# rawahars/CS744-Distributed-Data-Parallel

Hardware: AMD Instinct MI355X
Metric: images/sec (whole node) VGG-11 CIFAR-shaped at 1/2/4/8 MI355X; scaling eff (higher is better)
Workload: dtype fp32; 1 GPU; model=VGG-11, global_batch=256, local_batch=256, parallelism=dp1, comm=none, backend=native, device=mi355x, hipgraph=True, optimizer=SGD(lr=0.1, momentum=0.9, wd=1e-4), optimizer_overlap=False, early_buffer_broadcast=False, conv_gemm=f16x2

## Files before the change

### csrc/kernels/bwd_pair.h

```cpp
#pragma once
#include "conv_x3_body.h"
#include "wgrad_x3_body.h"

namespace cdp {
namespace pair_detail {

using namespace x3conv;
using namespace x3wgrad;

template <int DBM, int DBN, int WBM, int WBN>
struct PairCfg {
  static constexpr int kThreads = waves_m<DBM>() * 128;
  static_assert(kThreads == wg_threads<WBM>(), "both bodies must run the same workgroup size");
  static constexpr int kSmem = conv_x3_smem_elems<DBM, DBN, 2>() > wgrad_x3_smem_elems<WBM, WBN, 2, true>()
                                   ? conv_x3_smem_elems<DBM, DBN, 2>()
                                   : wgrad_x3_smem_elems<WBM, WBN, 2, true>();
};

template <int DBM, int DBN, int WBM, int WBN>
__global__ __launch_bounds__(waves_m<DBM>() * 128, DBM >= 256 ? 1 : 2) void bwd_pair_kernel(
    ConvGemmParams pd, WgradParams pw, int nd, int nw) {
  __shared__ __attribute__((aligned(16))) __bf16 smem[PairCfg<DBM, DBN, WBM, WBN>::kSmem];
  const int b = blockIdx.x;
  if (b < nd) conv_x3_body<DBM, DBN, 0, true, 2>(pd, smem, b, nd);
  else wgrad_x3_body<WBM, WBN, true, 2, true>(pw, smem, b - nd, nw);
}

template <int DBM, int DBN, int WBM, int WBN>
void launch_pair(const ConvGemmParams& pd, const WgradParams& pw, hipStream_t st) {
  const int nd = ((pd.M + DBM - 1) / DBM) * ((pd.Nout + DBN - 1) / DBN) * pd.splits;
  const int nw = ((pw.Cout + WBM - 1) / WBM) * ((pw.Kdim + WBN - 1) / WBN) * pw.splits;
  hipLaunchKernelGGL((bwd_pair_kernel<DBM, DBN, WBM, WBN>), dim3(nd + nw), dim3(PairCfg<DBM, DBN, WBM, WBN>::kThreads),
                     0, st, pd, pw, nd, nw);
}

template <int DBM, int DBN>
bool launch_pair_d(int wbm, int wbn, const ConvGemmParams& pd, const WgradParams& pw, hipStream_t st);
template <>
bool launch_pair_d<128, 128>(int, int, const ConvGemmParams&, const WgradParams&, hipStream_t);
template <>
bool launch_pair_d<128, 64>(int, int, const ConvGemmParams&, const WgradParams&, hipStream_t);
template <>
bool launch_pair_d<64, 128>(int, int, const ConvGemmParams&, const WgradParams&, hipStream_t);
template <>
bool launch_pair_d<64, 64>(int, int, const ConvGemmParams&, const WgradParams&, hipStream_t);

}
}

#define CDP_PAIR_TU(DBM, DBN)                                                                              \
  namespace cdp {                                                                                          \
  namespace pair_detail {                                                                                  \
  template <>                                                                                              \
  bool launch_pair_d<DBM, DBN>(int wbm, int wbn, const ConvGemmParams& pd, const WgradParams& pw,          \
                               hipStream_t st) {                                                           \
    if (wbm == 128 && wbn == 128) launch_pair<DBM, DBN, 128, 128>(pd, pw, st);                             \
    else if (wbm == 128 && wbn == 64) launch_pair<DBM, DBN, 128, 64>(pd, pw, st);                          \
    else if (wbm == 64 && wbn == 128) launch_pair<DBM, DBN, 64, 128>(pd, pw, st);                          \
    else if (wbm == 64 && wbn == 64) launch_pair<DBM, DBN, 64, 64>(pd, pw, st);                            \
    else return false;                                                                                     \
    return true;                                                                                           \
  }                                                                                                        \
  }                                                                                                        \
  }
```

### csrc/kernels/bwd_pair.hip

```cpp
#include "bwd_pair.h"

namespace cdp {

bool bwd_pair_ok(const ConvGemmParams& pd, int bm, int bn, const WgradParams& pw, int wbm, int wbn, int np) {
  if (np != 2 || (pd.C % 32) != 0 || (pd.Kdim % 32) != 0 || (pw.C % 4) != 0 || (pw.Cout % 4) != 0) return false;
  if (bm == 256) return bn == 128 && wbm == 256 && wbn == 128;
  return (bm == 64 || bm == 128) && (bn == 64 || bn == 128) && (wbm == 64 || wbm == 128) && (wbn == 64 || wbn == 128);
}

void bwd_pair_launch(const ConvGemmParams& pd, int bm, int bn, const WgradParams& pw, int wbm, int wbn,
                     hipStream_t st) {
  using namespace pair_detail;
  bool ok = false;
  if (bm == 256) {
    launch_pair<256, 128, 256, 128>(pd, pw, st);
    ok = true;
  } else if (bm == 128 && bn == 128) ok = launch_pair_d<128, 128>(wbm, wbn, pd, pw, st);
  else if (bm == 128 && bn == 64) ok = launch_pair_d<128, 64>(wbm, wbn, pd, pw, st);
  else if (bm == 64 && bn == 128) ok = launch_pair_d<64, 128>(wbm, wbn, pd, pw, st);
  else if (bm == 64 && bn == 64) ok = launch_pair_d<64, 64>(wbm, wbn, pd, pw, st);
  (void)ok;
}

}
```

### csrc/kernels/conv_x3.hip

```cpp
#include "conv_x3_body.h"

namespace cdp {

namespace {

using namespace x3conv;

template <int BM, int BN, int MODE, bool DGRAD, int NP = 3>
__global__ __launch_bounds__(waves_m<BM>() * 128, (NP == 2 && BM + BN <= 256) ? 2 : (BM + BN >= 256) ? 1 : 2) void
conv_x3_kernel(ConvGemmParams p) {
  __shared__ __attribute__((aligned(16))) __bf16 smem[conv_x3_smem_elems<BM, BN, NP>()];
  conv_x3_body<BM, BN, MODE, DGRAD, NP>(p, smem, blockIdx.x, gridDim.x);
}

template <int BM, int BN, int MODE, bool DGRAD>
void launch_x3(const ConvGemmParams& p, int ntiles, int np, hipStream_t st) {
  const dim3 blk(waves_m<BM>() * 128), grd(ntiles * p.splits);
  if (np == 1) hipLaunchKernelGGL((conv_x3_kernel<BM, BN, MODE, DGRAD, 1>), grd, blk, 0, st, p);
  else if (np == 2) hipLaunchKernelGGL((conv_x3_kernel<BM, BN, MODE, DGRAD, 2>), grd, blk, 0, st, p);
  else hipLaunchKernelGGL((conv_x3_kernel<BM, BN, MODE, DGRAD, 3>), grd, blk, 0, st, p);
}

template <int MODE, bool DGRAD>
void dispatch_x3(const ConvGemmParams& p, int bm, int bn, int np, hipStream_t st) {
  const int ntm = (p.M + bm - 1) / bm, ntn = (p.Nout + bn - 1) / bn;
  const int nt = ntm * ntn;
  if (bm == 256) launch_x3<256, 128, MODE, DGRAD>(p, nt, np, st);
  else if (bm == 128 && bn == 128) launch_x3<128, 128, MODE, DGRAD>(p, nt, np, st);
  else if (bm == 128 && bn == 64) launch_x3<128, 64, MODE, DGRAD>(p, nt, np, st);
  else if (bm == 64 && bn == 128) launch_x3<64, 128, MODE, DGRAD>(p, nt, np, st);
  else launch_x3<64, 64, MODE, DGRAD>(p, nt, np, st);
}

}

void conv_x3_launch(const ConvGemmParams& p, int bm, int bn, bool dgrad, hipStream_t st, int np) {
  if ((p.C % BK) == 0 && (p.Kdim % BK) == 0) {
    if (dgrad) dispatch_x3<0, true>(p, bm, bn, np, st);
    else dispatch_x3<0, false>(p, bm, bn, np, st);
  } else if ((p.C % 4) == 0 && (p.Kdim % 4) == 0) {
    if (dgrad) dispatch_x3<1, true>(p, bm, bn, np, st);
    else dispatch_x3<1, false>(p, bm, bn, np, st);
  } else {
    if (dgrad) dispatch_x3<2, true>(p, bm, bn, np, st);
    else dispatch_x3<2, false>(p, bm, bn, np, st);
  }
}

}
```

### csrc/kernels/conv_x3_body.h

```cpp
#pragma once
#include <type_traits>

#include "common.h"
#include "conv_epilogue.h"
#include "kernels.h"
#include "x3_common.h"

namespace cdp {
namespace x3conv {

constexpr int BK = 32;
constexpr int LDH = BK;

__device__ __forceinline__ int chunk_pos(int r, int c) { return c ^ ((-(r >> 2)) & 3); }

__device__ __forceinline__ void split8(const float (&v)[8], u32x4& s0, u32x4& s1, u32x4& s2) {
#pragma unroll
  for (int j = 0; j < 4; ++j) {
    unsigned a, b, c;
    split_pair(v[2 * j], v[2 * j + 1], a, b, c);
    s0[j] = a;
    s1[j] = b;
    s2[j] = c;
  }
// ... 1 lines not shown

__device__ __forceinline__ void split8h(const float (&v)[8], float s, u32x4& s0, u32x4& s1) {
#pragma unroll
  for (int j = 0; j < 4; ++j) {
    unsigned a, b;
    split_pair_h(v[2 * j], v[2 * j + 1], s, a, b);
    s0[j] = a;
    s1[j] = b;
  }
}

__device__ __forceinline__ u32x4 pack8(const float (&v)[8]) {
  u32x4 r;
#pragma unroll
  for (int j = 0; j < 4; ++j) r[j] = pack_bf16x2(f32x2{v[2 * j], v[2 * j + 1]});
  return r;
}

template <int BM, int BN, int NP>
constexpr int conv_x3_scales_at() {
  return 2 * NP * (BM + BN) * LDH > 2 * epi_lds_floats<BM, BN>() ? 2 * NP * (BM + BN) * LDH
                                                                  : 2 * epi_lds_floats<BM, BN>();
}
template <int BM, int BN, int NP>
constexpr int conv_x3_smem_elems() {
  return conv_x3_scales_at<BM, BN, NP>() + (NP == 2 ? 2 * (BM + BN) : 0);
}

template <int BM, int BN, int MODE, bool DGRAD, int NP = 3>
__device__ __forceinline__ void conv_x3_body(const ConvGemmParams& p, __bf16* __restrict__ smem, int vbid, int nvb) {
  static_assert(NP >= 1 && NP <= 3, "planes");
  constexpr unsigned ES = 2u;
  constexpr int WM = waves_m<BM>();
  constexpr int NT = WM * 128;
  constexpr int RS = NT / 4;
  constexpr int TM = BM / WM / 32;
  constexpr int TN = BN / 64;
  constexpr int A_LD = BM / RS;
  constexpr int B_LD = BN / RS;
  static_assert(A_LD >= 1 && B_LD >= 1, "tile too narrow for the loader");
  constexpr int PA = BM * LDH, PB = BN * LDH;
  constexpr int STAGE = NP * (PA + PB);

  const int tid = threadIdx.x;
  const int lane = tid & 63;
  const int wid = tid >> 6;
  const int wm = wid >> 1, wn = wid & 1;

  const int ntn = (p.Nout + BN - 1) / BN;
  const int bid = xcd_remap(vbid, nvb);
  const int tn_idx = bid % ntn;
  const int rest = bid / ntn;
  const int split = rest % p.splits;
  const int tm_idx = rest / p.splits;
// ... 321 lines not shown
      __syncthreads();
    }
    if (kt < kt_end) compute(smem);
  } else {
    finish_scales();
    publish_scales();
    __syncthreads();
  }

  if constexpr (NP == 2) {
#pragma unroll
    for (int b = 0; b < TN; ++b) {
      const float ib = s_ib[wn * (BN / 2) + b * 32 + l32];
#pragma unroll
      for (int a = 0; a < TM; ++a)
#pragma unroll
        for (int r = 0; r < 16; ++r)
          acc[a][b][r] = acc[a][b][r] * s_ia[wm * (BM / WM) + a * 32 + (r & 3) + 8 * (r >> 2) + 4 * hh] * ib;
    }
  }
  conv_epilogue<BM, BN>(p, acc, reinterpret_cast<float*>(smem), m0, n0, tm_idx, split);
}

}
}
```

### csrc/kernels/kernels.h

```cpp
#pragma once
#include <hip/hip_runtime.h>

#include "erase.h"
#include "lars.h"
#include "lr_sched.h"
#include "mix.h"
#include "rrc.h"

namespace cdp {

struct FastDiv {
  unsigned d, mul, shift;
};

inline FastDiv make_fastdiv(int d) {
  FastDiv f{(unsigned)d, 0u, 0u};
  if (d <= 1) return f;
  unsigned l = 0;
  while ((1ull << l) < (unsigned long long)d) ++l;
  const unsigned long long p = 31ull + l;
  f.mul = (unsigned)(((1ull << p) + (unsigned long long)d - 1ull) / (unsigned long long)d);
  f.shift = (unsigned)(p - 32ull);
  return f;
}
// ... 42 lines not shown

struct WgradParams {
  const float* dy;
  const float* x;
  float* out;
  int N, H, W, C, P, Q, KH, KW, stride, pad;
  int Cout, Kdim, M, splits;
  FastDiv fd_PQ, fd_Q, fd_C, fd_KW;
  const unsigned* dy_ch;
  const unsigned* x_ch;
};

constexpr int kActCopies = 8;
struct ActMaxOut {
  unsigned* img;
  unsigned* ch;
};
inline long long act_max_elems(long long N, long long C) { return N + kActCopies * C; }
inline long long weight_max_elems(long long Co, long long Ci) {
  return ((Ci + 31) / 32) * Co + ((Co + 31) / 32) * Ci;
}

void conv_igemm_launch(const ConvGemmParams& p, int bm, int bn, bool dgrad, hipStream_t st);
void conv_x3_launch(const ConvGemmParams& p, int bm, int bn, bool dgrad, hipStream_t st, int np = 3);
void splitk_reduce_launch(const float* slab, int S, int M, int Nout, const float* bias, float* y, float* part,
                          hipStream_t st, const RowRemap* rr = nullptr, const float* addend = nullptr);
int splitk_rows_per_part();

void wgrad_launch(const WgradParams& p, int bm, int bn, bool x3, hipStream_t st, int np = 3);
void act_max_launch(const float* x, int N, long long HW, int C, ActMaxOut o, hipStream_t st);
constexpr int kMaxAmaxSegs = 64;
struct WeightPrepArgs {
  const float* w[kMaxAmaxSegs];
  float* wt[kMaxAmaxSegs];
  int co[kMaxAmaxSegs], t[kMaxAmaxSegs], ci[kMaxAmaxSegs];
  int blk0[kMaxAmaxSegs + 1];
  long long pofs[kMaxAmaxSegs];
  int nseg;
};
void weight_prep_launch(const WeightPrepArgs& a, float* part, hipStream_t st);
struct SgdPrepSeg {
  long long off;
  float* wt;
  int co, t, ci, blk0;
  long long pofs;
};
struct SgdPrepChunk {
// ... 16 lines not shown
  long long* state = nullptr;
  const LrSchedCfg* cfg = nullptr;
  float* last_lr = nullptr;
  int advance = 0;
};
void sgd_prep_launch(float* p, const float* g, float* buf, const SgdPrepSeg* segs, int nseg, int nblk_w,
                     const SgdPrepChunk* chunks, int nchunk, float* wmax, const float* lr_ptr, float lr,
                     float momentum, float dampening, float wd, float grad_scale, bool nesterov, bool first,
                     bool maximize, hipStream_t st, long long* counter = nullptr, const ClipArgs& clip = ClipArgs{},
                     const LarsArgs& lars = LarsArgs{}, const EmaArgs& ema = EmaArgs{},
                     const SchedArgs& sched = SchedArgs{});
void slab_sum_launch(const float* slab, int S, long long n, float* dst, bool accumulate, hipStream_t st);
void slab_sum_strided_launch(const float* slab, int S, long long n_src, int src_cols, int dst_cols, float* dst,
                             bool accumulate, hipStream_t st);

bool stem_ok(int Cin, int KH, int KW, int stride, int pad, int Co);
void stem_fwd_launch(const float* x, const float* w, const float* bias, float* y, float* part, int N, int H, int W,
                     int Cin, int Co, hipStream_t st);
int stem_wgrad_blocks(int N, int H, int W);
void stem_wgrad_launch(const float* y, const float* gout, const float* stats, const float* sums, const float* x,
                       float* slab, int nblk, int N, int H, int W, int Cin, hipStream_t st);

bool bwd_pair_ok(const ConvGemmParams& pd, int bm, int bn, const WgradParams& pw, int wbm, int wbn, int np);
void bwd_pair_launch(const ConvGemmParams& pd, int bm, int bn, const WgradParams& pw, int wbm, int wbn,
                     hipStream_t st);

struct BwdReduceArgs {
  const float* d_slab;
  float* d_y;
  const float* d_addend;
  int d_S, d_M, d_Nout;
  const float* bn_y;
  const float* bn_stats;
  float* bn_part;
  int bn_H, bn_W, bn_pool, bn_relu, bn_ps;
  FastDiv bn_fd_wo, bn_fd_ho;
  const float4* w_slab;
  float4* w_dst;
  int w_S;
  long long w_n4;
  int nbd, d_nbx, w_cb;
};
void bwd_reduce_launch(BwdReduceArgs a, hipStream_t st);
int bwd_reduce_rows_per_part();

int bn_bwd_grid(int N, int H, int W, int C, bool pool);
void bn_finalize_launch(const float* part, int nparts, int rpp, int M, int C, const float* gamma, const float* beta,
                        float* running_mean, float* running_var, long long* nbt, float momentum, float eps,
// ... 119 lines not shown
```

### csrc/runtime/bindings.cpp

```cpp
#include <torch/csrc/utils/pybind.h>
#include <torch/extension.h>

#include <execinfo.h>
#include <signal.h>
#include <unistd.h>

#include "ops.h"
#include "rccl_comm.h"
#include "reducer.h"

namespace py = pybind11;
using namespace cdp;

namespace {
void segv_backtrace(int sig) {
  void* frames[64];
  const int n = backtrace(frames, 64);
  const char msg[] = "[cdp] native backtrace:\n";
  (void)!write(2, msg, sizeof(msg) - 1);
  backtrace_symbols_fd(frames, n, 2);
  signal(sig, SIG_DFL);
  raise(sig);
}
}

PYBIND11_MODULE(_C, m) {
  if (const char* bt = std::getenv("CDP_SEGV_BT"); bt && bt[0] == '1') signal(SIGSEGV, segv_backtrace);
  m.doc() = "cs744_distributed_data_parallel_amd native runtime (gfx950 kernels, RCCL comm, reducer)";
  m.attr("ARCH") = "gfx950";

  m.def("set_conv_gemm", &set_conv_gemm, py::arg("mode"),
        "select the conv GEMM engine: x3 (3-term bf16 split), f16x2 (scaled 2-term fp16 split), f32 (exact fp32 "
        "MFMA) or bf16 (bf16 operands, non-parity)");
  m.def("get_conv_gemm", &get_conv_gemm);
  m.def("set_gemm_override", &set_gemm_override, py::arg("kind"), py::arg("bm") = 0, py::arg("bn") = 0,
        py::arg("splits") = 0, "force the tile / split-K plan of later GEMMs (tuning sweeps; zeros restore the planner)");
  m.def("pair_launches", &pair_launches, "paired data/weight-gradient launches issued so far");
  m.def("plan_info", &plan_info, py::arg("kind"), py::arg("M"), py::arg("N"), py::arg("K"));
  m.def("clear_hip_error", [] { return std::string(hipGetErrorName(hipGetLastError())); },
        "reset the thread's last HIP error (e.g. after an invalidated stream capture) and return its name");
  m.def("conv2d_fwd", &conv2d_fwd, py::arg("x"), py::arg("w"), py::arg("bias"), py::arg("stride"), py::arg("pad"),
        py::arg("want_stats") = false, py::arg("x_amax") = py::none(), py::arg("w_amax") = py::none());
  m.def("conv2d_dgrad", &conv2d_dgrad, py::arg("dy"), py::arg("w"), py::arg("in_shape"), py::arg("stride"),
        py::arg("pad"), py::arg("addend") = py::none(), py::arg("dy_amax") = py::none(), py::arg("w_amax") = py::none(),
        py::arg("w_t") = py::none());
  m.def("conv2d_wgrad", &conv2d_wgrad, py::arg("dy"), py::arg("x"), py::arg("w_shape"), py::arg("stride"),
        py::arg("pad"), py::arg("out") = py::none(), py::arg("accumulate") = false, py::arg("dy_amax") = py::none(),
        py::arg("x_amax") = py::none());
  m.def("conv_bn_act_fwd", &conv_bn_act_fwd, py::arg("x"), py::arg("w"), py::arg("b"), py::arg("gamma"),
        py::arg("beta"), py::arg("running_mean"), py::arg("running_var"), py::arg("num_batches_tracked"),
        py::arg("momentum"), py::arg("eps"), py::arg("training"), py::arg("stride"), py::arg("pad"), py::arg("pool"),
        py::arg("relu"), py::arg("residual"), py::arg("x_amax") = py::none(), py::arg("w_amax") = py::none(),
        py::arg("res_y") = py::none(), py::arg("res_stats") = py::none(), py::arg("defer_apply") = false,
        "fused conv + BN [+ residual] [+ ReLU] [+ 2x2 max-pool] forward; returns (out, y, stats, x_saved, out_amax, "
        "x_amax, w_amax, relu_mask). defer_apply: statistics only, out a shape-only placeholder; res_y / res_stats: "
        "the residual as such a deferred branch's raw output and stats, normalized inside this block's apply pass");
  m.def("act_max", &act_max_of, py::arg("t"),
        "f16x2 engine: an activation's per-image / per-channel |max| slots by the standalone pass (int32 [N + "
        "copies * C], float bits; undefined tensor for other engines)");
  m.def("act_max_memsets", &act_max_memsets, "slot-chunk memsets issued so far (tests)");
// ... 266 lines not shown
```

### csrc/runtime/ops.cpp

```cpp
#include "ops.h"

#include <c10/hip/HIPCachingAllocator.h>
#include <c10/hip/HIPFunctions.h>
#include <c10/hip/HIPGuard.h>
#include <c10/hip/HIPStream.h>
#include <torch/extension.h>

#include <algorithm>
#include <array>
#include <atomic>
#include <cstdlib>
#include <cstring>
#include <functional>
#include <mutex>
#include <tuple>
#include <string>
#include <unordered_map>

#include "../kernels/adam.h"
#include "../kernels/kernels.h"

namespace cdp {

namespace {
// ... 352 lines not shown
  std::lock_guard<std::mutex> g(gemm_log_mu());
  gemm_log_vec().push_back({kind, M, N, K, bm, bn, splits});
}
std::vector<std::tuple<std::string, int64_t, int64_t, int64_t, int64_t, int64_t, int64_t>> gemm_log_snapshot(bool clear) {
  std::lock_guard<std::mutex> g(gemm_log_mu());
  std::vector<std::tuple<std::string, int64_t, int64_t, int64_t, int64_t, int64_t, int64_t>> out;
  for (const auto& r : gemm_log_vec()) out.emplace_back(r.kind, r.M, r.N, r.K, r.bm, r.bn, r.splits);
  if (clear) gemm_log_vec().clear();
  return out;
}
static void wgrad_launch_logged(const WgradParams& p, int bm, int bn, bool x3, hipStream_t st, int np) {
  gemm_log_add("wgrad", p.Cout, p.Kdim, (long long)p.M, bm, bn, p.splits);
  wgrad_launch(p, bm, bn, x3, st, np);
}

static bool narrow_stores() {
  static const bool on = [] {
    const char* e = std::getenv("CDP_WIDE_STORES");
    return e && e[0] == '0';
  }();
  return on;
}

void conv_launch(const ConvGemmParams& p0, int bm, int bn, bool dgrad, hipStream_t st) {
  gemm_log_add(dgrad ? "dgrad" : "fwd", p0.M, p0.Nout, p0.Kdim, bm, bn, p0.splits);
  ConvGemmParams p = p0;
  p.narrow = narrow_stores();
  if (x3_family() && x3_ok(p, dgrad)) {
    TORCH_CHECK(!f16x2_mode() || (p.a_img && p.b_row), "f16x2 conv GEMM launched without operand maxima");
    conv_x3_launch(p, bm, bn, dgrad, st, split_planes());
  }
  else conv_igemm_launch(p, bm, bn, dgrad, st);
}

struct DeferredReduce {
  at::Tensor w_slab;
  float* w_dst = nullptr;
  int w_S = 0;
  long long w_n = 0;
  at::Tensor d_slab;
  const float* d_src = nullptr;
  float* d_y = nullptr;
  const float* d_addend = nullptr;
  int d_S = 0, d_M = 0, d_Nout = 0;
  bool d_on = false;
};

struct PendingWgrad {
  bool set = false;
  WgradParams p{};
  int bm = 0, bn = 0;
  std::function<void()> after;
  std::vector<at::Tensor> keep;
// ... 17 lines not shown

bool bwd_fuse_enabled() {
  static const bool on = [] {
    const char* e = std::getenv("CDP_BWD_FUSE");
    return !(e && e[0] == '0');
  }();
  return on;
}

std::atomic<long long>& pair_counter() {
  static std::atomic<long long> n{0};
  return n;
}

void conv_launch_or_pair(const ConvGemmParams& p, const GemmPlan& g, bool dgrad, hipStream_t st,
                         PendingWgrad* pending) {
  if (pending && pending->set && dgrad && f16x2_mode() && x3_ok(p, true) && p.a_img && p.b_row &&
      bwd_pair_ok(p, g.bm, g.bn, pending->p, pending->bm, pending->bn, split_planes())) {
    gemm_log_add("pair_dgrad", p.M, p.Nout, p.Kdim, g.bm, g.bn, p.splits);
    gemm_log_add("pair_wgrad", pending->p.Cout, pending->p.Kdim, (long long)pending->p.M, pending->bm, pending->bn,
                 pending->p.splits);
    ConvGemmParams q = p;
    q.narrow = narrow_stores();
    bwd_pair_launch(q, g.bm, g.bn, pending->p, pending->bm, pending->bn, st);
    pair_counter().fetch_add(1, std::memory_order_relaxed);
    pending->run_after();
    return;
  }
  conv_launch(p, g.bm, g.bn, dgrad, st);
}

int conv_gemm_splitk(ConvGemmParams p, const GemmPlan& g, bool dgrad, hipStream_t st, at::TensorOptions opts,
                     std::vector<at::Tensor>& keep, const std::function<float*(int)>& alloc_part = nullptr,
                     DeferredReduce* defer = nullptr, PendingWgrad* pending = nullptr) {
  p.splits = g.splits;
  if (g.splits == 1) {
    if (alloc_part) p.part = alloc_part(g.bm);
    conv_launch_or_pair(p, g, dgrad, st, pending);
    if (defer && !alloc_part && !p.part && !p.bias && !p.rr.on && !p.addend && (p.Nout % 4) == 0) {
      defer->d_on = true;
      defer->d_src = p.y;
      defer->d_y = p.y;
      defer->d_addend = nullptr;
      defer->d_S = 1;
      defer->d_M = p.M;
      defer->d_Nout = p.Nout;
    }
    return g.bm;
// ... 309 lines not shown
}

at::Tensor pad_channels4(const at::Tensor& t, at::Tensor* amax = nullptr) {
  const int64_t C = t.size(1), C4 = (C + 3) / 4 * 4;
  at::Tensor o = at::empty({t.size(0), C4, t.size(2), t.size(3)}, t.options().memory_format(at::MemoryFormat::ChannelsLast));
  if (C < 4 && t.is_contiguous(at::MemoryFormat::ChannelsLast)) {
    hipStream_t st = cur_stream();
    ActMaxOut am{nullptr, nullptr};
    if (amax) {
      *amax = new_act_max(t.size(0), 4, t, st);
      am = act_out(*amax, t.size(0));
    }
    pad_c4_launch(t.data_ptr<float>(), (int)t.size(0), t.size(2) * t.size(3), (int)C, o.data_ptr<float>(), am, st);
    return o;
  }
  o.zero_();
  o.narrow(1, 0, C).copy_(t);
  return o;
}

}

int64_t pair_launches() { return pair_counter().load(std::memory_order_relaxed); }

void set_gemm_override(const std::string& kind, int64_t bm, int64_t bn, int64_t splits) {
  TORCH_CHECK(kind == "conv" || kind == "wgrad", "set_gemm_override: kind must be 'conv' or 'wgrad'");
  TORCH_CHECK(bm == 0 || bm == 64 || bm == 128 || bm == 256, "bm must be 0, 64, 128 or 256");
  TORCH_CHECK(bn == 0 || bn == 64 || bn == 128, "bn must be 0, 64 or 128");
  TORCH_CHECK(bm != 256 || bn == 128, "256-row tiles are 256x128");
  PlanOverride& o = kind == "conv" ? conv_override() : wgrad_override();
  o.bm = (int)bm;
  o.bn = (int)bn;
  o.splits = (int)splits;
}

std::vector<int64_t> plan_info(const std::string& kind, int64_t M, int64_t N, int64_t K) {
  if (kind == "conv" || kind == "dgrad") {
    const GemmPlan g = plan_gemm(M, (int)N, (int)K, kind == "dgrad" ? 1 : 0);
    return {g.bm, g.bn, g.splits};
  }
  TORCH_CHECK(kind == "wgrad", "plan_info: kind must be 'conv', 'dgrad' or 'wgrad'");
  const WgradPlan w = plan_wgrad((int)N, (int)K, M);
  return {w.bm, w.bn, w.splits};
}

void set_conv_gemm(const std::string& mode) {
// ... 1651 lines not shown
```

### csrc/runtime/ops.h

```cpp
#pragma once
#include <ATen/ATen.h>
#include <c10/util/Optional.h>

#include <string>
#include <tuple>
#include <vector>

namespace cdp {

void set_conv_gemm(const std::string& mode);
int64_t pair_launches();
void set_gemm_override(const std::string& kind, int64_t bm, int64_t bn, int64_t splits);
std::vector<int64_t> plan_info(const std::string& kind, int64_t M, int64_t N, int64_t K);
std::string get_conv_gemm();
std::vector<at::Tensor> conv2d_fwd(const at::Tensor& x, const at::Tensor& w, const c10::optional<at::Tensor>& bias,
                                   int64_t stride, int64_t pad, bool want_stats,
                                   const c10::optional<at::Tensor>& x_amax = c10::nullopt,
                                   const c10::optional<at::Tensor>& w_amax = c10::nullopt);
at::Tensor conv2d_dgrad(const at::Tensor& dy, const at::Tensor& w, std::vector<int64_t> in_shape, int64_t stride,
                        int64_t pad, const c10::optional<at::Tensor>& addend,
                        const c10::optional<at::Tensor>& dy_amax = c10::nullopt,
                        const c10::optional<at::Tensor>& w_amax = c10::nullopt,
                        const c10::optional<at::Tensor>& w_t = c10::nullopt);
at::Tensor conv2d_wgrad(const at::Tensor& dy, const at::Tensor& x, std::vector<int64_t> w_shape, int64_t stride,
                        int64_t pad, const c10::optional<at::Tensor>& out, bool accumulate,
                        const c10::optional<at::Tensor>& dy_amax = c10::nullopt,
                        const c10::optional<at::Tensor>& x_amax = c10::nullopt);
at::Tensor conv2d_wgrad_keep(const at::Tensor& dy, const at::Tensor& x, std::vector<int64_t> w_shape, int64_t stride,
                             int64_t pad, const c10::optional<at::Tensor>& out, bool accumulate, int64_t keep_c,
                             const c10::optional<at::Tensor>& dy_amax = c10::nullopt,
                             const c10::optional<at::Tensor>& x_amax = c10::nullopt);
std::vector<at::Tensor> conv_bn_act_fwd(const at::Tensor& x, const at::Tensor& w, const c10::optional<at::Tensor>& b,
                                        const c10::optional<at::Tensor>& gamma, const c10::optional<at::Tensor>& beta,
                                        const c10::optional<at::Tensor>& running_mean,
// ... 167 lines not shown
```

Baseline: 199,100 images/sec.

## Add tap-reuse main loop for 3x3 conv GEMMs on small feature maps

Adds a specialized conv main loop for 3x3 stride-1 pad-1 convolutions whose whole output image fits in an M tile. It loads each activation channel chunk into LDS once and reuses it across all nine filter taps by shifting rows, instead of re-gathering the im2col tile for every tap. The loop is wired into the plain conv launch and the paired dgrad/wgrad kernel, and is on by default where a heuristic says it pays. The cost is extra LDS for a zero row, a more complex tap/row indexing path, and added template instantiations.

Result: no change. 200,600 images/sec (median of 6 runs) (+0.8%).

```diff
diff --git a/csrc/kernels/bwd_pair.h b/csrc/kernels/bwd_pair.h
--- a/csrc/kernels/bwd_pair.h
+++ b/csrc/kernels/bwd_pair.h
@@ -8,42 +8,56 @@
 using namespace x3conv;
 using namespace x3wgrad;
 
-template <int DBM, int DBN, int WBM, int WBN>
+template <int DBM, int DBN, int WBM, int WBN, bool TR = false>
 struct PairCfg {
   static constexpr int kThreads = waves_m<DBM>() * 128;
   static_assert(kThreads == wg_threads<WBM>(), "both bodies must run the same workgroup size");
-  static constexpr int kSmem = conv_x3_smem_elems<DBM, DBN, 2>() > wgrad_x3_smem_elems<WBM, WBN, 2, true>()
-                                   ? conv_x3_smem_elems<DBM, DBN, 2>()
+  static constexpr int kSmem = conv_x3_smem_elems<DBM, DBN, 2, TR>() > wgrad_x3_smem_elems<WBM, WBN, 2, true>()
+                                   ? conv_x3_smem_elems<DBM, DBN, 2, TR>()
                                    : wgrad_x3_smem_elems<WBM, WBN, 2, true>();
 };
 
-template <int DBM, int DBN, int WBM, int WBN>
+template <int DBM, int DBN, int WBM, int WBN, bool TR = false>
 __global__ __launch_bounds__(waves_m<DBM>() * 128, DBM >= 256 ? 1 : 2) void bwd_pair_kernel(
     ConvGemmParams pd, WgradParams pw, int nd, int nw) {
-  __shared__ __attribute__((aligned(16))) __bf16 smem[PairCfg<DBM, DBN, WBM, WBN>::kSmem];
+  __shared__ __attribute__((aligned(16))) __bf16 smem[PairCfg<DBM, DBN, WBM, WBN, TR>::kSmem];
   const int b = blockIdx.x;
-  if (b < nd) conv_x3_body<DBM, DBN, 0, true, 2>(pd, smem, b, nd);
+  if (b < nd) conv_x3_body<DBM, DBN, 0, true, 2, TR>(pd, smem, b, nd);
   else wgrad_x3_body<WBM, WBN, true, 2, true>(pw, smem, b - nd, nw);
 }
 
-template <int DBM, int DBN, int WBM, int WBN>
+template <int DBM, int DBN, int WBM, int WBN, bool TR = false>
 void launch_pair(const ConvGemmParams& pd, const WgradParams& pw, hipStream_t st) {
   const int nd = ((pd.M + DBM - 1) / DBM) * ((pd.Nout + DBN - 1) / DBN) * pd.splits;
   const int nw = ((pw.Cout + WBM - 1) / WBM) * ((pw.Kdim + WBN - 1) / WBN) * pw.splits;
-  hipLaunchKernelGGL((bwd_pair_kernel<DBM, DBN, WBM, WBN>), dim3(nd + nw), dim3(PairCfg<DBM, DBN, WBM, WBN>::kThreads),
-                     0, st, pd, pw, nd, nw);
+  hipLaunchKernelGGL((bwd_pair_kernel<DBM, DBN, WBM, WBN, TR>), dim3(nd + nw),
+                     dim3(PairCfg<DBM, DBN, WBM, WBN, TR>::kThreads), 0, st, pd, pw, nd, nw);
 }
 
 template <int DBM, int DBN>
-bool launch_pair_d(int wbm, int wbn, const ConvGemmParams& pd, const WgradParams& pw, hipStream_t st);
+constexpr bool pair_tr_built() { return !(DBM == 128 && DBN == 64); }
+
+template <int DBM, int DBN, int WBM, int WBN>
+void launch_pair_tr(bool tr, const ConvGemmParams& pd, const WgradParams& pw, hipStream_t st) {
+  if constexpr (pair_tr_built<DBM, DBN>()) {
+    if (tr) {
+      launch_pair<DBM, DBN, WBM, WBN, true>(pd, pw, st);
+      return;
+    }
+  }
+  launch_pair<DBM, DBN, WBM, WBN>(pd, pw, st);
+}
+
+template <int DBM, int DBN>
+bool launch_pair_d(int wbm, int wbn, bool tr, const ConvGemmParams& pd, const WgradParams& pw, hipStream_t st);
 template <>
-bool launch_pair_d<128, 128>(int, int, const ConvGemmParams&, const WgradParams&, hipStream_t);
+bool launch_pair_d<128, 128>(int, int, bool, const ConvGemmParams&, const WgradParams&, hipStream_t);
 template <>
-bool launch_pair_d<128, 64>(int, int, const ConvGemmParams&, const WgradParams&, hipStream_t);
+bool launch_pair_d<128, 64>(int, int, bool, const ConvGemmParams&, const WgradParams&, hipStream_t);
 template <>
-bool launch_pair_d<64, 128>(int, int, const ConvGemmParams&, const WgradParams&, hipStream_t);
+bool launch_pair_d<64, 128>(int, int, bool, const ConvGemmParams&, const WgradParams&, hipStream_t);
 template <>
-bool launch_pair_d<64, 64>(int, int, const ConvGemmParams&, const WgradParams&, hipStream_t);
+bool launch_pair_d<64, 64>(int, int, bool, const ConvGemmParams&, const WgradParams&, hipStream_t);
 
 }
 }
@@ -52,12 +66,12 @@
   namespace cdp {                                                                                          \
   namespace pair_detail {                                                                                  \
   template <>                                                                                              \
-  bool launch_pair_d<DBM, DBN>(int wbm, int wbn, const ConvGemmParams& pd, const WgradParams& pw,          \
+  bool launch_pair_d<DBM, DBN>(int wbm, int wbn, bool tr, const ConvGemmParams& pd, const WgradParams& pw, \
                                hipStream_t st) {                                                           \
-    if (wbm == 128 && wbn == 128) launch_pair<DBM, DBN, 128, 128>(pd, pw, st);                             \
-    else if (wbm == 128 && wbn == 64) launch_pair<DBM, DBN, 128, 64>(pd, pw, st);                          \
-    else if (wbm == 64 && wbn == 128) launch_pair<DBM, DBN, 64, 128>(pd, pw, st);                          \
-    else if (wbm == 64 && wbn == 64) launch_pair<DBM, DBN, 64, 64>(pd, pw, st);                            \
+    if (wbm == 128 && wbn == 128) launch_pair_tr<DBM, DBN, 128, 128>(tr, pd, pw, st);                      \
+    else if (wbm == 128 && wbn == 64) launch_pair_tr<DBM, DBN, 128, 64>(tr, pd, pw, st);                   \
+    else if (wbm == 64 && wbn == 128) launch_pair_tr<DBM, DBN, 64, 128>(tr, pd, pw, st);                   \
+    else if (wbm == 64 && wbn == 64) launch_pair_tr<DBM, DBN, 64, 64>(tr, pd, pw, st);                     \
     else return false;                                                                                     \
     return true;                                                                                           \
   }                                                                                                        \
diff --git a/csrc/kernels/bwd_pair.hip b/csrc/kernels/bwd_pair.hip
--- a/csrc/kernels/bwd_pair.hip
+++ b/csrc/kernels/bwd_pair.hip
@@ -8,17 +8,20 @@
   return (bm == 64 || bm == 128) && (bn == 64 || bn == 128) && (wbm == 64 || wbm == 128) && (wbn == 64 || wbn == 128);
 }
 
+bool bwd_pair_has_tap_reuse(int bm, int bn) { return !(bm == 128 && bn == 64); }
+
 void bwd_pair_launch(const ConvGemmParams& pd, int bm, int bn, const WgradParams& pw, int wbm, int wbn,
-                     hipStream_t st) {
+                     hipStream_t st, bool tap_reuse) {
   using namespace pair_detail;
+  const bool tr = tap_reuse && bwd_pair_has_tap_reuse(bm, bn) && conv_tap_reuse_ok(pd, bm, true, 2);
   bool ok = false;
   if (bm == 256) {
-    launch_pair<256, 128, 256, 128>(pd, pw, st);
+    launch_pair_tr<256, 128, 256, 128>(tr, pd, pw, st);
     ok = true;
-  } else if (bm == 128 && bn == 128) ok = launch_pair_d<128, 128>(wbm, wbn, pd, pw, st);
-  else if (bm == 128 && bn == 64) ok = launch_pair_d<128, 64>(wbm, wbn, pd, pw, st);
-  else if (bm == 64 && bn == 128) ok = launch_pair_d<64, 128>(wbm, wbn, pd, pw, st);
-  else if (bm == 64 && bn == 64) ok = launch_pair_d<64, 64>(wbm, wbn, pd, pw, st);
+  } else if (bm == 128 && bn == 128) ok = launch_pair_d<128, 128>(wbm, wbn, tr, pd, pw, st);
+  else if (bm == 128 && bn == 64) ok = launch_pair_d<128, 64>(wbm, wbn, tr, pd, pw, st);
+  else if (bm == 64 && bn == 128) ok = launch_pair_d<64, 128>(wbm, wbn, tr, pd, pw, st);
+  else if (bm == 64 && bn == 64) ok = launch_pair_d<64, 64>(wbm, wbn, tr, pd, pw, st);
   (void)ok;
 }
 
diff --git a/csrc/kernels/conv_x3.hip b/csrc/kernels/conv_x3.hip
--- a/csrc/kernels/conv_x3.hip
+++ b/csrc/kernels/conv_x3.hip
@@ -6,44 +6,60 @@
 
 using namespace x3conv;
 
-template <int BM, int BN, int MODE, bool DGRAD, int NP = 3>
+template <int BM, int BN, int MODE, bool DGRAD, int NP = 3, bool TR = false>
 __global__ __launch_bounds__(waves_m<BM>() * 128, (NP == 2 && BM + BN <= 256) ? 2 : (BM + BN >= 256) ? 1 : 2) void
 conv_x3_kernel(ConvGemmParams p) {
-  __shared__ __attribute__((aligned(16))) __bf16 smem[conv_x3_smem_elems<BM, BN, NP>()];
-  conv_x3_body<BM, BN, MODE, DGRAD, NP>(p, smem, blockIdx.x, gridDim.x);
+  __shared__ __attribute__((aligned(16))) __bf16 smem[conv_x3_smem_elems<BM, BN, NP, TR>()];
+  conv_x3_body<BM, BN, MODE, DGRAD, NP, TR>(p, smem, blockIdx.x, gridDim.x);
 }
 
 template <int BM, int BN, int MODE, bool DGRAD>
-void launch_x3(const ConvGemmParams& p, int ntiles, int np, hipStream_t st) {
+void launch_x3(const ConvGemmParams& p, int ntiles, int np, bool tr, hipStream_t st) {
   const dim3 blk(waves_m<BM>() * 128), grd(ntiles * p.splits);
+  if constexpr (MODE == 0) {
+    if (tr && np == 2) {
+      hipLaunchKernelGGL((conv_x3_kernel<BM, BN, 0, DGRAD, 2, true>), grd, blk, 0, st, p);
+      return;
+    }
+  }
   if (np == 1) hipLaunchKernelGGL((conv_x3_kernel<BM, BN, MODE, DGRAD, 1>), grd, blk, 0, st, p);
   else if (np == 2) hipLaunchKernelGGL((conv_x3_kernel<BM, BN, MODE, DGRAD, 2>), grd, blk, 0, st, p);
   else hipLaunchKernelGGL((conv_x3_kernel<BM, BN, MODE, DGRAD, 3>), grd, blk, 0, st, p);
 }
 
 template <int MODE, bool DGRAD>
-void dispatch_x3(const ConvGemmParams& p, int bm, int bn, int np, hipStream_t st) {
+void dispatch_x3(const ConvGemmParams& p, int bm, int bn, int np, bool tr, hipStream_t st) {
   const int ntm = (p.M + bm - 1) / bm, ntn = (p.Nout + bn - 1) / bn;
   const int nt = ntm * ntn;
-  if (bm == 256) launch_x3<256, 128, MODE, DGRAD>(p, nt, np, st);
-  else if (bm == 128 && bn == 128) launch_x3<128, 128, MODE, DGRAD>(p, nt, np, st);
-  else if (bm == 128 && bn == 64) launch_x3<128, 64, MODE, DGRAD>(p, nt, np, st);
-  else if (bm == 64 && bn == 128) launch_x3<64, 128, MODE, DGRAD>(p, nt, np, st);
-  else launch_x3<64, 64, MODE, DGRAD>(p, nt, np, st);
+  if (bm == 256) launch_x3<256, 128, MODE, DGRAD>(p, nt, np, tr, st);
+  else if (bm == 128 && bn == 128) launch_x3<128, 128, MODE, DGRAD>(p, nt, np, tr, st);
+  else if (bm == 128 && bn == 64) launch_x3<128, 64, MODE, DGRAD>(p, nt, np, tr, st);
+  else if (bm == 64 && bn == 128) launch_x3<64, 128, MODE, DGRAD>(p, nt, np, tr, st);
+  else launch_x3<64, 64, MODE, DGRAD>(p, nt, np, tr, st);
 }
 
 }
 
-void conv_x3_launch(const ConvGemmParams& p, int bm, int bn, bool dgrad, hipStream_t st, int np) {
+bool conv_tap_reuse_ok(const ConvGemmParams& p, int bm, bool dgrad, int np) {
+  if (np != 2 || (p.C % BK) != 0 || p.Kdim != 9 * p.C) return false;
+  if (p.KH != 3 || p.KW != 3 || p.stride != 1 || p.pad != 1 || (dgrad && p.pad_w != 1)) return false;
+  if (p.P != p.H || p.Q != p.W || p.rr.on) return false;
+  const int pq = p.P * p.Q;
+  if (pq <= 0 || pq > bm || (bm % pq) != 0) return false;
+  return p.splits >= 1 && p.splits <= p.C / BK;
+}
+
+void conv_x3_launch(const ConvGemmParams& p, int bm, int bn, bool dgrad, hipStream_t st, int np, bool tap_reuse) {
   if ((p.C % BK) == 0 && (p.Kdim % BK) == 0) {
-    if (dgrad) dispatch_x3<0, true>(p, bm, bn, np, st);
-    else dispatch_x3<0, false>(p, bm, bn, np, st);
+    const bool tr = tap_reuse && conv_tap_reuse_ok(p, bm, dgrad, np);
+    if (dgrad) dispatch_x3<0, true>(p, bm, bn, np, tr, st);
+    else dispatch_x3<0, false>(p, bm, bn, np, tr, st);
   } else if ((p.C % 4) == 0 && (p.Kdim % 4) == 0) {
-    if (dgrad) dispatch_x3<1, true>(p, bm, bn, np, st);
-    else dispatch_x3<1, false>(p, bm, bn, np, st);
+    if (dgrad) dispatch_x3<1, true>(p, bm, bn, np, false, st);
+    else dispatch_x3<1, false>(p, bm, bn, np, false, st);
   } else {
-    if (dgrad) dispatch_x3<2, true>(p, bm, bn, np, st);
-    else dispatch_x3<2, false>(p, bm, bn, np, st);
+    if (dgrad) dispatch_x3<2, true>(p, bm, bn, np, false, st);
+    else dispatch_x3<2, false>(p, bm, bn, np, false, st);
   }
 }
 
diff --git a/csrc/kernels/conv_x3_body.h b/csrc/kernels/conv_x3_body.h
--- a/csrc/kernels/conv_x3_body.h
+++ b/csrc/kernels/conv_x3_body.h
@@ -47,14 +47,22 @@
   return 2 * NP * (BM + BN) * LDH > 2 * epi_lds_floats<BM, BN>() ? 2 * NP * (BM + BN) * LDH
                                                                   : 2 * epi_lds_floats<BM, BN>();
 }
-template <int BM, int BN, int NP>
+template <int BM, int BN, int NP, bool TR = false>
 constexpr int conv_x3_smem_elems() {
-  return conv_x3_scales_at<BM, BN, NP>() + (NP == 2 ? 2 * (BM + BN) : 0);
-}
-
-template <int BM, int BN, int MODE, bool DGRAD, int NP = 3>
+  return conv_x3_scales_at<BM, BN, NP>() + (NP == 2 ? 2 * (BM + BN) : 0) + (TR ? 4 * LDH : 0);
+}
+
+template <int BM, int BN, bool DGRAD>
+__device__ __forceinline__ void conv_x3_tr_body(const ConvGemmParams& p, __bf16* __restrict__ smem, int vbid, int nvb);
+
+template <int BM, int BN, int MODE, bool DGRAD, int NP = 3, bool TR = false>
 __device__ __forceinline__ void conv_x3_body(const ConvGemmParams& p, __bf16* __restrict__ smem, int vbid, int nvb) {
   static_assert(NP >= 1 && NP <= 3, "planes");
+  if constexpr (TR) {
+    static_assert(NP == 2 && MODE == 0, "tap reuse: f16x2, whole K-tiles per tap");
+    conv_x3_tr_body<BM, BN, DGRAD>(p, smem, vbid, nvb);
+    return;
+  }
   constexpr unsigned ES = 2u;
   constexpr int WM = waves_m<BM>();
   constexpr int NT = WM * 128;
@@ -422,5 +430,294 @@
   conv_epilogue<BM, BN>(p, acc, reinterpret_cast<float*>(smem), m0, n0, tm_idx, split);
 }
 
-}
-}
+template <int BM, int BN, bool DGRAD>
+__device__ __forceinline__ void conv_x3_tr_body(const ConvGemmParams& p, __bf16* __restrict__ smem, int vbid, int nvb) {
+  constexpr int NP = 2;
+  constexpr unsigned ES = 2u;
+  constexpr int WM = waves_m<BM>();
+  constexpr int NT = WM * 128;
+  constexpr int RS = NT / 4;
+  constexpr int TM = BM / WM / 32;
+  constexpr int TN = BN / 64;
+  constexpr int A_LD = BM / RS;
+  constexpr int B_LD = BN / RS;
+  static_assert(A_LD >= 1 && A_LD <= 3 && B_LD >= 1, "tile outside the loader's range");
+  constexpr int PA = BM * LDH, PB = BN * LDH;
+  constexpr int ASLOT = NP * PA;
+  constexpr int BSTAGE = NP * PB;
+  constexpr int B_AT = 2 * ASLOT;
+  constexpr int Z_AT = conv_x3_scales_at<BM, BN, NP>() + 2 * (BM + BN);
+  static_assert((ASLOT & (ASLOT - 1)) == 0 && ASLOT % 128 == 0 && Z_AT % 128 == 0, "slot toggle / zeros' banks");
+  static_assert(B_AT + 2 * BSTAGE <= conv_x3_scales_at<BM, BN, NP>(), "operands run into the scales");
+  constexpr int NTAP = 9;
+
+  const int tid = threadIdx.x;
+  const int lane = tid & 63;
+  const int wid = tid >> 6;
+  const int wm = wid >> 1, wn = wid & 1;
+  const int l32 = lane & 31;
+  const int hh = lane >> 5;
+
+  const int ntn = (p.Nout + BN - 1) / BN;
+  const int bid = xcd_remap(vbid, nvb);
+  const int tn_idx = bid % ntn;
+  const int rest = bid / ntn;
+  const int split = rest % p.splits;
+  const int tm_idx = rest / p.splits;
+  const int m0 = tm_idx * BM, n0 = tn_idx * BN;
+  const int nch = p.C / BK;
+  const int ch_begin = (int)(((long long)split * nch) / p.splits);
+  const int ch_end = (int)(((long long)(split + 1) * nch) / p.splits);
+  const int nt = (ch_end - ch_begin) * NTAP;
+  const int PQ = p.P * p.Q;
+
+  const int kq = (tid & 3) * 8;
+  const int rrow = tid >> 2;
+
+  const unsigned xplane = ((unsigned)p.N * (unsigned)(p.H * p.W * p.C)) << ES;
+  const unsigned wplane = ((unsigned)p.Nout * (unsigned)p.Kdim) << ES;
+  const __amdgpu_buffer_rsrc_t xr = make_rsrc(p.x, xplane);
+  const __amdgpu_buffer_rsrc_t wr = make_rsrc(p.w, wplane);
+
+  unsigned a_off[A_LD], a_io[A_LD];
+#pragma unroll
+  for (int i = 0; i < A_LD; ++i) {
+    const int m = m0 + rrow + RS * i;
+    const bool ok = m < p.M;
+    const int n = fdiv(ok ? m : 0, p.fd_PQ);
+    a_io[i] = ok ? (unsigned)n * 4u : kOOB;
+    a_off[i] = ok ? ((unsigned)m * (unsigned)p.C + (unsigned)kq) << ES : kOOB;
+  }
+  unsigned b_off[B_LD];
+#pragma unroll
+  for (int i = 0; i < B_LD; ++i) {
+    const int n = n0 + rrow + RS * i;
+    b_off[i] = n < p.Nout ? (unsigned)(mul24(n, p.Kdim) + kq) << ES : kOOB;
+  }
+
+  constexpr int BQ = 4;
+  float sa_r[A_LD], sb_r[B_LD];
+  unsigned am_a[A_LD];
+  float am_b[B_LD][BQ];
+  const __amdgpu_buffer_rsrc_t brow = make_rsrc(p.b_row, (unsigned)p.b_np * (unsigned)p.b_stride * 4u);
+  {
+    const __amdgpu_buffer_rsrc_t ir = make_rsrc(p.a_img, (unsigned)p.N * 4u);
+#pragma unroll
+    for (int i = 0; i < A_LD; ++i) am_a[i] = __builtin_amdgcn_raw_buffer_load_b32(ir, (int)a_io[i], 0, 0);
+#pragma unroll
+    for (int i = 0; i < B_LD; ++i) {
+      const int n = n0 + rrow + RS * i;
+#pragma unroll
+      for (int j = 0; j < BQ; ++j) {
+        const int q = (tid & 3) + 4 * j;
+        const unsigned o = (n < p.Nout && q < p.b_np) ? (unsigned)(q * p.b_stride + n) * 4u : kOOB;
+        am_b[i][j] = __uint_as_float(__builtin_amdgcn_raw_buffer_load_b32(brow, (int)o, 0, 0));
+      }
+    }
+  }
+  auto finish_scales = [&]() {
+#pragma unroll
+    for (int i = 0; i < A_LD; ++i) sa_r[i] = pow2_scale(__uint_as_float(am_a[i]));
+#pragma unroll
+    for (int i = 0; i < B_LD; ++i) {
+      const int n = n0 + rrow + RS * i;
+      float m = 0.f;
+#pragma unroll
+      for (int j = 0; j < BQ; ++j) m = fmaxf(m, am_b[i][j]);
+      for (int q = (tid & 3) + 4 * BQ; q < p.b_np; q += 4) {
+        const unsigned o = n < p.Nout ? (unsigned)(q * p.b_stride + n) * 4u : kOOB;
+        m = fmaxf(m, __uint_as_float(__builtin_amdgcn_raw_buffer_load_b32(brow, (int)o, 0, 0)));
+      }
+      m = fmaxf(m, __shfl_xor(m, 1, kWave));
+      m = fmaxf(m, __shfl_xor(m, 2, kWave));
+      sb_r[i] = pow2_scale(m);
+    }
+  };
+
+  int f_row[TM];
+  unsigned f_taps[TM];
+#pragma unroll
+  for (int a = 0; a < TM; ++a) {
+    const int r = wm * (BM / WM) + a * 32 + l32;
+    const int rem = r - mul24(fdiv(r, p.fd_PQ), PQ);
+    const int pp = fdiv(rem, p.fd_Q);
+    const int qq = rem - mul24(pp, p.Q);
+    unsigned mk = 0;
+#pragma unroll
+    for (int kh = 0; kh < 3; ++kh)
+#pragma unroll
+      for (int kw = 0; kw < 3; ++kw) {
+        const int sh = DGRAD ? pp + p.pad - kh : pp - p.pad + kh;
+        const int sw = DGRAD ? qq + p.pad_w - kw : qq - p.pad + kw;
+        if ((unsigned)sh < (unsigned)p.H && (unsigned)sw < (unsigned)p.W) mk |= 1u << (kh * 3 + kw);
+      }
+    f_row[a] = r;
+    f_taps[a] = mk;
+  }
+
+  float va[A_LD][8];
+  float vb0[B_LD][8], vb1[B_LD][8];
+
+  auto put4 = [](float (&d)[8], int off, float4 v) {
+    d[off] = v.x;
+    d[off + 1] = v.y;
+    d[off + 2] = v.z;
+    d[off + 3] = v.w;
+  };
+  auto load_a = [&](int ch, bool valid) {
+#pragma unroll
+    for (int i = 0; i < A_LD; ++i) {
+      const unsigned o = valid ? a_off[i] + ((unsigned)(ch * BK) << ES) : kOOB;
+      put4(va[i], 0, bload4(xr, o));
+      put4(va[i], 4, bload4(xr, o + 16u));
+    }
+  };
+  auto load_b = [&](int tap, int ch, auto& vb, bool valid) {
+    const unsigned r0 = (unsigned)(mul24(tap, p.C) + ch * BK) << ES;
+#pragma unroll
+    for (int i = 0; i < B_LD; ++i) {
+      const unsigned o = valid ? b_off[i] + r0 : kOOB;
+      put4(vb[i], 0, bload4(wr, o));
+      put4(vb[i], 4, bload4(wr, o + 16u));
+    }
+  };
+  const int cp = chunk_pos(rrow, tid & 3) * 8;
+  auto store_a_row = [&](int i, int slot) {
+    __bf16* d = smem + slot + (rrow + RS * i) * LDH + cp;
+    u32x4 s0, s1;
+    split8h(va[i], sa_r[i], s0, s1);
+    *reinterpret_cast<u32x4*>(d) = s0;
+    *reinterpret_cast<u32x4*>(d + PA) = s1;
+  };
+  auto store_b = [&](const auto& vb, __bf16* st) {
+#pragma unroll
+    for (int i = 0; i < B_LD; ++i) {
+      __bf16* d = st + (rrow + RS * i) * LDH + cp;
+      u32x4 s0, s1;
+      split8h(vb[i], sb_r[i], s0, s1);
+      *reinterpret_cast<u32x4*>(d) = s0;
+      *reinterpret_cast<u32x4*>(d + PB) = s1;
+    }
+  };
+
+  f32x16 acc[TM][TN];
+#pragma unroll
+  for (int a = 0; a < TM; ++a)
+#pragma unroll
+    for (int b = 0; b < TN; ++b)
+#pragma unroll
+      for (int r = 0; r < 16; ++r) acc[a][b][r] = 0.f;
+
+  auto compute = [&](int slot, const __bf16* bs, int tap) {
+    const int kh = (tap * 11) >> 5, kw = tap - 3 * kh;
+    const int shift = DGRAD ? (p.pad - kh) * p.W + (p.pad_w - kw) : (kh - p.pad) * p.W + (kw - p.pad);
+    const unsigned tbit = 1u << tap;
+    int o0[TM], o1[TM];
+#pragma unroll
+    for (int a = 0; a < TM; ++a) {
+      const bool ok = (f_taps[a] & tbit) != 0u;
+      const int rr = f_row[a] + shift;
+      const int o = rr * LDH + chunk_pos(rr, hh) * 8;
+      const int z = Z_AT + (o & 127);
+      o0[a] = ok ? slot + o : z;
+      o1[a] = ok ? slot + PA + o : z;
+    }
+#pragma unroll
+    for (int s = 0; s < 2; ++s) {
+      f16x8 af[TM][2], bf[TN][2];
+#pragma unroll
+      for (int a = 0; a < TM; ++a) {
+        af[a][0] = *reinterpret_cast<const f16x8*>(smem + (o0[a] ^ (16 * s)));
+        af[a][1] = *reinterpret_cast<const f16x8*>(smem + (o1[a] ^ (16 * s)));
+      }
+#pragma unroll
+      for (int b = 0; b < TN; ++b) {
+        const int r = wn * (BN / 2) + b * 32 + l32;
+        const __bf16* src = bs + r * LDH + chunk_pos(r, 2 * s + hh) * 8;
+#pragma unroll
+        for (int q = 0; q < 2; ++q) bf[b][q] = *reinterpret_cast<const f16x8*>(src + q * PB);
+      }
+#pragma unroll
+      for (int a = 0; a < TM; ++a)
+#pragma unroll
+        for (int b = 0; b < TN; ++b) {
+          f32x16 c = acc[a][b];
+          c = __builtin_amdgcn_mfma_f32_32x32x16_f16(af[a][1], bf[b][0], c, 0, 0, 0);
+          c = __builtin_amdgcn_mfma_f32_32x32x16_f16(af[a][0], bf[b][1], c, 0, 0, 0);
+          c = __builtin_amdgcn_mfma_f32_32x32x16_f16(af[a][0], bf[b][0], c, 0, 0, 0);
+          acc[a][b] = c;
+        }
+    }
+  };
+
+  float* s_ia = reinterpret_cast<float*>(smem + conv_x3_scales_at<BM, BN, NP>());
+  float* s_ib = s_ia + BM;
+  auto publish_scales = [&]() {
+    if ((tid & 3) == 0) {
+#pragma unroll
+      for (int i = 0; i < A_LD; ++i) s_ia[rrow + RS * i] = 1.f / sa_r[i];
+#pragma unroll
+      for (int i = 0; i < B_LD; ++i) s_ib[rrow + RS * i] = 1.f / sb_r[i];
+    }
+  };
+
+  __bf16* const bst0 = smem + B_AT;
+  __bf16* const bst1 = smem + B_AT + BSTAGE;
+  if (nt > 0) {
+    load_a(ch_begin, true);
+    load_b(0, ch_begin, vb0, true);
+    load_b(1, ch_begin, vb1, true);
+    finish_scales();
+    publish_scales();
+    if (tid < 16) *reinterpret_cast<u32x4*>(smem + Z_AT + tid * 8) = u32x4{0u, 0u, 0u, 0u};
+#pragma unroll
+    for (int i = 0; i < A_LD; ++i) store_a_row(i, 0);
+    store_b(vb0, bst0);
+    __syncthreads();
+    int c_tap = 0, c_ch = ch_begin, c_slot = 0;
+    int l_tap = 2, l_ch = ch_begin;
+    auto step = [&](int t, auto& vload, const auto& vstore, const __bf16* bcur, __bf16* bnext) {
+      load_b(l_tap, l_ch, vload, t + 2 < nt);
+      if (c_tap == 0) load_a(c_ch + 1, c_ch + 1 < ch_end);
+      compute(c_slot, bcur, c_tap);
+      store_b(vstore, bnext);
+#pragma unroll
+      for (int i = 0; i < A_LD; ++i)
+        if (c_tap == 2 + 2 * i) store_a_row(i, c_slot ^ ASLOT);
+      __syncthreads();
+      if (++c_tap == NTAP) {
+        c_tap = 0;
+        ++c_ch;
+        c_slot ^= ASLOT;
+      }
+      if (++l_tap == NTAP) {
+        l_tap = 0;
+        ++l_ch;
+      }
+    };
+    int t = 0;
+    for (; t + 1 < nt; t += 2) {
+      step(t, vb0, vb1, bst0, bst1);
+      step(t + 1, vb1, vb0, bst1, bst0);
+    }
+    if (t < nt) compute(c_slot, bst0, c_tap);
+  } else {
+    finish_scales();
+    publish_scales();
+    __syncthreads();
+  }
+
+#pragma unroll
+  for (int b = 0; b < TN; ++b) {
+    const float ib = s_ib[wn * (BN / 2) + b * 32 + l32];
+#pragma unroll
+    for (int a = 0; a < TM; ++a)
+#pragma unroll
+      for (int r = 0; r < 16; ++r)
+        acc[a][b][r] = acc[a][b][r] * s_ia[wm * (BM / WM) + a * 32 + (r & 3) + 8 * (r >> 2) + 4 * hh] * ib;
+  }
+  conv_epilogue<BM, BN>(p, acc, reinterpret_cast<float*>(smem), m0, n0, tm_idx, split);
+}
+
+}
+}
diff --git a/csrc/kernels/kernels.h b/csrc/kernels/kernels.h
--- a/csrc/kernels/kernels.h
+++ b/csrc/kernels/kernels.h
@@ -88,7 +88,9 @@
 }
 
 void conv_igemm_launch(const ConvGemmParams& p, int bm, int bn, bool dgrad, hipStream_t st);
-void conv_x3_launch(const ConvGemmParams& p, int bm, int bn, bool dgrad, hipStream_t st, int np = 3);
+void conv_x3_launch(const ConvGemmParams& p, int bm, int bn, bool dgrad, hipStream_t st, int np = 3,
+                    bool tap_reuse = false);
+bool conv_tap_reuse_ok(const ConvGemmParams& p, int bm, bool dgrad, int np);
 void splitk_reduce_launch(const float* slab, int S, int M, int Nout, const float* bias, float* y, float* part,
                           hipStream_t st, const RowRemap* rr = nullptr, const float* addend = nullptr);
 int splitk_rows_per_part();
@@ -151,8 +153,9 @@
                        float* slab, int nblk, int N, int H, int W, int Cin, hipStream_t st);
 
 bool bwd_pair_ok(const ConvGemmParams& pd, int bm, int bn, const WgradParams& pw, int wbm, int wbn, int np);
+bool bwd_pair_has_tap_reuse(int bm, int bn);
 void bwd_pair_launch(const ConvGemmParams& pd, int bm, int bn, const WgradParams& pw, int wbm, int wbn,
-                     hipStream_t st);
+                     hipStream_t st, bool tap_reuse = false);
 
 struct BwdReduceArgs {
   const float* d_slab;
diff --git a/csrc/runtime/bindings.cpp b/csrc/runtime/bindings.cpp
--- a/csrc/runtime/bindings.cpp
+++ b/csrc/runtime/bindings.cpp
@@ -36,6 +36,9 @@
   m.def("set_gemm_override", &set_gemm_override, py::arg("kind"), py::arg("bm") = 0, py::arg("bn") = 0,
         py::arg("splits") = 0, "force the tile / split-K plan of later GEMMs (tuning sweeps; zeros restore the planner)");
   m.def("pair_launches", &pair_launches, "paired data/weight-gradient launches issued so far");
+  m.def("tap_reuse_launches", &tap_reuse_launches, "conv GEMM launches that ran the tap-reuse main loop so far");
+  m.def("set_tap_reuse", &set_tap_reuse, py::arg("on"),
+        "tap-reuse conv main loop: 0 off, 1 every eligible GEMM, 2 where it pays (default), -1 follow CDP_TAP_REUSE");
   m.def("plan_info", &plan_info, py::arg("kind"), py::arg("M"), py::arg("N"), py::arg("K"));
   m.def("clear_hip_error", [] { return std::string(hipGetErrorName(hipGetLastError())); },
         "reset the thread's last HIP error (e.g. after an invalidated stream capture) and return its name");
diff --git a/csrc/runtime/ops.cpp b/csrc/runtime/ops.cpp
--- a/csrc/runtime/ops.cpp
+++ b/csrc/runtime/ops.cpp
@@ -398,13 +398,36 @@
   return on;
 }
 
+int& tap_reuse_override() {
+  static int v = -1;
+  return v;
+}
+int tap_reuse_mode() {
+  if (tap_reuse_override() >= 0) return tap_reuse_override();
+  const char* e = std::getenv("CDP_TAP_REUSE");
+  return e && e[0] == '0' ? 0 : e && e[0] == '1' ? 1 : 2;
+}
+bool tap_reuse_pays(const ConvGemmParams& p, int bm, int bn) {
+  return p.splits >= 1 && ((p.C / 32) % p.splits) == 0 && p.P * p.Q >= 16 && bm >= bn;
+}
+bool tap_reuse_for(const ConvGemmParams& p, int bm, int bn, bool dgrad) {
+  const int mode = tap_reuse_mode();
+  return mode != 0 && conv_tap_reuse_ok(p, bm, dgrad, split_planes()) && (mode == 1 || tap_reuse_pays(p, bm, bn));
+}
+std::atomic<long long>& tap_reuse_counter() {
+  static std::atomic<long long> n{0};
+  return n;
+}
+
 void conv_launch(const ConvGemmParams& p0, int bm, int bn, bool dgrad, hipStream_t st) {
   gemm_log_add(dgrad ? "dgrad" : "fwd", p0.M, p0.Nout, p0.Kdim, bm, bn, p0.splits);
   ConvGemmParams p = p0;
   p.narrow = narrow_stores();
   if (x3_family() && x3_ok(p, dgrad)) {
     TORCH_CHECK(!f16x2_mode() || (p.a_img && p.b_row), "f16x2 conv GEMM launched without operand maxima");
-    conv_x3_launch(p, bm, bn, dgrad, st, split_planes());
+    const bool tr = tap_reuse_for(p, bm, bn, dgrad);
+    conv_x3_launch(p, bm, bn, dgrad, st, split_planes(), tr);
+    if (tr) tap_reuse_counter().fetch_add(1, std::memory_order_relaxed);
   }
   else conv_igemm_launch(p, bm, bn, dgrad, st);
 }
@@ -468,8 +491,10 @@
                  pending->p.splits);
     ConvGemmParams q = p;
     q.narrow = narrow_stores();
-    bwd_pair_launch(q, g.bm, g.bn, pending->p, pending->bm, pending->bn, st);
+    const bool tr = bwd_pair_has_tap_reuse(g.bm, g.bn) && tap_reuse_for(q, g.bm, g.bn, true);
+    bwd_pair_launch(q, g.bm, g.bn, pending->p, pending->bm, pending->bn, st, tr);
     pair_counter().fetch_add(1, std::memory_order_relaxed);
+    if (tr) tap_reuse_counter().fetch_add(1, std::memory_order_relaxed);
     pending->run_after();
     return;
   }
@@ -825,6 +850,8 @@
 }
 
 int64_t pair_launches() { return pair_counter().load(std::memory_order_relaxed); }
+int64_t tap_reuse_launches() { return tap_reuse_counter().load(std::memory_order_relaxed); }
+void set_tap_reuse(int64_t on) { tap_reuse_override() = on < 0 ? -1 : on > 2 ? 2 : (int)on; }
 
 void set_gemm_override(const std::string& kind, int64_t bm, int64_t bn, int64_t splits) {
   TORCH_CHECK(kind == "conv" || kind == "wgrad", "set_gemm_override: kind must be 'conv' or 'wgrad'");
diff --git a/csrc/runtime/ops.h b/csrc/runtime/ops.h
--- a/csrc/runtime/ops.h
+++ b/csrc/runtime/ops.h
@@ -10,6 +10,8 @@
 
 void set_conv_gemm(const std::string& mode);
 int64_t pair_launches();
+int64_t tap_reuse_launches();
+void set_tap_reuse(int64_t on);
 void set_gemm_override(const std::string& kind, int64_t bm, int64_t bn, int64_t splits);
 std::vector<int64_t> plan_info(const std::string& kind, int64_t M, int64_t N, int64_t K);
 std::string get_conv_gemm();
```
